# CloudEngineHub/MARL-LLM

Measured on AMD Instinct MI355X. Metric: agent-steps/sec, higher is better.
Workload: dtype f64 (state, every index / flag / reward decision) + f32 (obs, prior, action I/O, pre-filters); 1 GPU; assembly env, 64 agents x 4096 envs per GPU (64 x 4096 total), assembled state, prior-policy actions; agents=64, envs_per_gpu=4096, envs_total=4096, obs_dtype=f32, state_dtype=f64, seed=226, parallelism=env-sharded x1, no collective on the step path

## Files before the change

### marl_llm_amd/csrc/env_api.hip

```cpp

#include <hip/hip_runtime.h>

#include <algorithm>
#include <cmath>
#include <cstddef>
#include <cstdint>
#include <cstring>
#include <new>
#include <string>
#include <utility>
#include <vector>

#include "swarm_env.h"
#include "env_types.h"

using namespace swarm_internal;

namespace {

thread_local std::string g_create_error;

double cut_le(double t) { return cut_lt(std::nextafter(t, INFINITY)); }

int npad_for(int n)
{
    int v = 8;
    while (v < n) v <<= 1;
    return v;
}

int step_launch(swarm_env *h, const Pass &ps)
{
    return h->cfg.large_swarm ? large_launch(h, ps) : env_launch(h, ps);
}

bool detect_lattice(const double *gx, const double *gy, int n, LatEnv &L)
{
    if (n < 2) return false;
    double l2 = INFINITY; int k0 = -1;
    for (int c = 0; c + 1 < n; ++c) {
        const double dx = gx[c + 1] - gx[c], dy = gy[c + 1] - gy[c], d2 = dx * dx + dy * dy;
        if (d2 < l2) { l2 = d2; k0 = c; }
    }
    if (!(l2 > 0) || k0 < 0) return false;
    double cand[4][2]; int ncand = 0;
    for (int c = 0; c + 1 < n && ncand < 4; ++c) {
        const double dx = gx[c + 1] - gx[c], dy = gy[c + 1] - gy[c], d2 = dx * dx + dy * dy;
        if (d2 > l2 * (1.0 + 1e-6)) continue;
        bool seen = false;
        for (int q = 0; q < ncand; ++q)
            if (std::fabs(cand[q][0] - dx) + std::fabs(cand[q][1] - dy) < 1e-6 * std::sqrt(l2)) seen = true;
        if (!seen) { cand[ncand][0] = dx; cand[ncand][1] = dy; ++ncand; }
    }
    std::vector<int> ai((size_t)n), bi((size_t)n);
    double ux = 0, uy = 0, vx = 0, vy = 0;
    bool found = false;
    for (int q = 0; q < ncand && !found; ++q) {
        ux = cand[q][0]; uy = cand[q][1]; vx = -uy; vy = ux;
        for (int pass = 0; pass < 2 && !found; ++pass) {
            bool ok = true;
            for (int c = 0; c < n && ok; ++c) {
                const double rx = gx[c] - gx[0], ry = gy[c] - gy[0];
                const double a = (rx * ux + ry * uy) / l2, b = (rx * vx + ry * vy) / l2;
                const double ar = std::nearbyint(a), br = std::nearbyint(b);
                if (std::fabs(a - ar) > 1e-6 || std::fabs(b - br) > 1e-6 || std::fabs(ar) > 4096 || std::fabs(br) > 4096) ok = false;
                ai[(size_t)c] = (int)ar; bi[(size_t)c] = (int)br;
            }
            if (!ok) break;
            bool order = true, flip = false;
            for (int c = 0; c + 1 < n; ++c) {
                if (bi[(size_t)c + 1] == bi[(size_t)c]) { if (ai[(size_t)c + 1] <= ai[(size_t)c]) order = false; }
                else if (bi[(size_t)c + 1] < bi[(size_t)c]) { flip = true; order = false; }
            }
            if (order) { found = true; break; }
            if (pass == 0 && flip) { vx = -vx; vy = -vy; continue; }
            break;
        }
    }
    if (!found) return false;
    int amin = ai[0], amax = ai[0], bmin = bi[0], bmax = bi[0];
    for (int c = 0; c < n; ++c) {
        amin = std::min(amin, ai[(size_t)c]); amax = std::max(amax, ai[(size_t)c]);
        bmin = std::min(bmin, bi[(size_t)c]); bmax = std::max(bmax, bi[(size_t)c]);
    }
    if (amax - amin + 1 > 64 || bmax - bmin + 1 > 64) return false;
    std::memset(&L, 0, sizeof(L));
    L.ncols = amax - amin + 1; L.nrows = bmax - bmin + 1;
    for (int b = 0; b < 64; ++b) L.rowstart[b] = 0;
    int prev_b = -1;
    for (int c = 0; c < n; ++c) {
        const int a = ai[(size_t)c] - amin, b = bi[(size_t)c] - bmin;
        if (b != prev_b) { if (b < prev_b) return false; L.rowstart[b] = (short)c; prev_b = b; }
        if (L.rowmask[b] & (1ull << a)) return false;
        L.rowmask[b] |= 1ull << a;
    }
    L.ox = gx[0] - (ai[0] - amin) * ux - (bi[0] - bmin) * vx;
    L.oy = gy[0] - (ai[0] - amin) * uy - (bi[0] - bmin) * vy;
    L.uxi = ux / l2; L.uyi = uy / l2; L.vxi = vx / l2; L.vyi = vy / l2;
    const double l = std::sqrt(l2);
    L.R = (float)l;
    return true;
}

int window_rows(float R) { return (int)std::floor(2.0f * (R + 0.01f)) + 1; }

void set_lattice_mode(swarm_env *h, bool any_walk, bool any_scan, float rmax, float cmax, int ncols_max)
{
    KP &k = h->kp;
    if (h->cfg.large_swarm) {
        h->path_mode = PATH_SCAN; h->half = false; k.lattice = 0; k.path_filter = 0;
        return;
    }
    k.lat_n32 = ncols_max <= 32 ? 1 : 0;
    k.lat_rw = (int)std::ceil(rmax + 0.02f);
    k.lat_cw = (int)std::ceil(cmax + 0.02f);
    k.lat_nrs = window_rows(rmax); k.lat_nrc = window_rows(cmax);
    const bool demote = (h->cfg.debug_flags & 8) != 0;
    h->path_mode = (!any_walk || h->lattice_disabled || k.lat_nrs > 15 || (any_scan && demote)) ? PATH_SCAN : any_scan ? PATH_MIXED : PATH_WALK;
    k.lattice = h->path_mode != PATH_SCAN ? 1 : 0;
    k.path_filter = 0;
    {
        const double dx = 1.2e-5, R = std::fmax(1.0, (double)rmax), thr = 0.05 * R / k.d_sen;
        const double dpsi_R = 2.4675 * 2.0 * std::sqrt(2.0) * dx + 1.2e-6 * R;
        k.rew_ga_lat = (float)(1.3 * (dpsi_R + dx + thr * dpsi_R / R));
        k.rew_gb_lat = (float)(4e-6 * R / k.d_sen);
    }
    {
        const int epb_full = env_geometry(h->npad, false).envs;
        const long long grid_full = ((long long)h->cfg.n_env + epb_full - 1) / epb_full;
        h->half = h->path_mode == PATH_WALK && h->npad < 64 && epb_full >= 2 && !(h->cfg.debug_flags & 4) && 2 * grid_full <= (long long)h->n_cu * 6;
    }
    env_layout(k, h->npad, h->half);
}

int export_pass(swarm_env *h, bool lists, bool cap_even)
{
    if (lists && !h->d_exp_occ) {
        const size_t EN = (size_t)h->cfg.n_env * h->cfg.n_agents;
        DevBuf<int> sensed, occ;
        HIP_ALLOC(h, sensed, EN * (size_t)h->kp.g_max);
        HIP_ALLOC(h, occ, EN * (size_t)h->kp.occ_max);
        h->d_exp_sensed = std::move(sensed); h->d_exp_occ = std::move(occ);
    }
    Pass ps;
    ps.export_small = true; ps.export_lists = lists; ps.cap_even = cap_even;
    return step_launch(h, ps);
}

LatInfo classify_cells(const swarm_env *h, const double *gx, const double *gy, int n, LatEnv &L)
{
    std::memset(&L, 0, sizeof(L));
    if (h->lattice_disabled || !detect_lattice(gx, gy, n, L)) {
        std::memset(&L, 0, sizeof(L));
        return LatInfo{false, false, true, 0.0f, 0.0f, 0};
    }
    const double l = L.R;
    L.R = (float)(h->kp.d_sen / l); L.Rc = (float)((h->kp.r_avoid / 2.0) / l);
    const LatInfo info = {true, window_rows(L.R) <= 15, window_rows(L.R) > 15, L.R, L.Rc, L.ncols};
    if (!info.walk) std::memset(&L, 0, sizeof(L));
    return info;
}

LatInfo lattice_summary(const LatInfo *first, const LatInfo *last)
{
    LatInfo m = {true, false, false, 0.0f, 0.0f, 0};
    for (; first != last; ++first) {
        m.ok = m.ok && first->ok; m.scan = m.scan || first->scan;
        if (!first->walk) continue;
        m.walk = true;
        m.R = std::max(m.R, first->R); m.Rc = std::max(m.Rc, first->Rc);
        m.ncols = std::max(m.ncols, first->ncols);
    }
    return m;
}

LatInfo lattice_mode_of(swarm_env *h, const LatInfo *first, const LatInfo *last)
{
    const LatInfo m = lattice_summary(first, last);
    set_lattice_mode(h, m.walk, m.scan, m.R, m.Rc, m.ncols);
    return m;
}

ShapeSet shape_set(const swarm_env *h)
{
    ShapeSet S;
    S.n_shapes = h->n_shapes; S.cells = h->d_shape_cells.get(); S.n_g = h->d_shape_ng.get(); S.l_cell = h->d_shape_l.get();
    S.c_in = h->d_shape_cin.get(); S.lat = h->d_shape_lat.get();
    return S;
}

int interleave(swarm_env *h, int e0, int count)
{
    HIP_LAUNCHED(h, launch_interleave(h->stream, h->d_cells.get(), h->d_cells_xy.get(), h->kp.ng_max, e0, count));
    return SWARM_OK;
}

bool rule_tiled(const swarm_env *h)
{
    return h->cfg.n_agents > 256 || (!h->cfg.large_swarm && (h->cfg.debug_flags & 32) != 0);
}

}

int swarm_internal::fail(swarm_env *h, int code, const std::string &msg)
{
    if (h) h->err = msg; else g_create_error = msg;
    return code;
}

int swarm_internal_env_info(const swarm_env_t *h, swarm_env_info *out)
{
    if (!h || !out) return SWARM_ERR_INVALID;
    out->device = h->device; out->n_env = h->cfg.n_env; out->n_agents = h->cfg.n_agents; out->obs_dim = h->kp.obs_dim;
    out->obs_dtype = h->cfg.obs_dtype; out->with_prior = h->cfg.with_prior != 0; out->observed = h->observed;
    out->g_max = h->kp.g_max; out->llm_action = h->cfg.llm_action != 0; out->n_shapes = h->n_shapes;
    out->large_swarm = h->cfg.large_swarm != 0;
    out->rule_tiled = rule_tiled(h);
    return SWARM_OK;
}

int swarm_internal_metrics_step(swarm_env_t *h, double *out)
{
    if (!h || !out) return SWARM_ERR_INVALID;
    if (!h->have_cells || !h->have_state) return fail(h, SWARM_ERR_STATE, "swarm_rollout_eval: cells / state not set");
    DeviceGuard g(h->device);
    HIP_LAUNCHED(h, launch_metrics_step(h->stream, h->kp, h->n_cu, out));
    return SWARM_OK;
}

int swarm_internal_expert_view(swarm_env_t *h, bool lists, swarm_expert_view *out)
{
    if (!h || !out) return SWARM_ERR_INVALID;
    if (lists) {
        if (!h->d_act64) HIP_ALLOC(h, h->d_act64, (size_t)h->cfg.n_env * h->cfg.n_agents);
        const int rc = export_pass(h, true, true);
        if (rc != SWARM_OK) return rc;
    }
    out->p = h->d_p.get(); out->dp = h->d_dp.get(); out->cells = h->d_cells.get();
    out->near_cell = h->d_near.get(); out->in_flag = h->d_inflag.get(); out->exp_sensed = h->d_exp_sensed.get();
    out->act_next = h->d_act_next.get(); out->act64 = h->d_act64.get();
    out->d_sen = h->kp.d_sen; out->r_avoid = h->kp.r_avoid;
    out->n_env = h->cfg.n_env; out->n_agents = h->cfg.n_agents; out->g_max = h->kp.g_max; out->ng_max = h->kp.ng_max;
    return SWARM_OK;
}

extern "C" {

int swarm_abi_version(void) { return SWARM_ABI_VERSION; }

void swarm_default_config(swarm_config_t *c)
{
    if (!c) return;
    std::memset(c, 0, sizeof(*c));
    c->n_env = 1; c->n_agents = 30; c->n_cells_max = 576;
    c->topo_nei_max = 6; c->num_obs_grid_max = 80; c->num_occupied_grid_max = 200;
    c->is_boundary = 1; c->with_self_state = 1; c->with_prior = 1;
    c->obs_dtype = SWARM_F32; c->device = -1;
    c->d_sen = 0.4; c->r_avoid = 0.15; c->size_a = 0.035;
    c->k_ball = 30; c->k_wall = 100; c->c_wall = 5; c->vel_max = 0.8; c->dt = 0.1;
    c->boundary[0] = -2.4; c->boundary[1] = 2.4; c->boundary[2] = 2.4; c->boundary[3] = -2.4;
    c->prior_gain[0] = 2.0; c->prior_gain[1] = 3.0; c->prior_gain[2] = 2.0;
    c->llm_repulsion = 1.0; c->llm_action = 0;
}

const char *swarm_last_error(const swarm_env_t *h) { return h ? h->err.c_str() : g_create_error.c_str(); }

int swarm_create(const swarm_config_t *cfg, swarm_env_t **out)
{
    if (!cfg || !out) return fail(nullptr, SWARM_ERR_INVALID, "swarm_create: null argument");
    *out = nullptr;
    if (cfg->n_env < 1) return fail(nullptr, SWARM_ERR_INVALID, "n_env must be >= 1");
    if (cfg->large_swarm != 0 && cfg->large_swarm != 1) return fail(nullptr, SWARM_ERR_INVALID, "large_swarm must be 0 or 1");
    if (cfg->large_swarm) {
        if (cfg->n_agents < 1 || cfg->n_agents > 1024) return fail(nullptr, SWARM_ERR_INVALID, "n_agents must be in [1, 1024] (large_swarm)");
    } else if (cfg->n_agents < 1 || cfg->n_agents > 256) return fail(nullptr, SWARM_ERR_INVALID, "n_agents must be in [1, 256]");
    if (cfg->n_cells_max < 1 || cfg->n_cells_max > 32767) return fail(nullptr, SWARM_ERR_INVALID, "n_cells_max must be in [1, 32767]");
    if (cfg->topo_nei_max < 1 || cfg->topo_nei_max > kTopoMax) return fail(nullptr, SWARM_ERR_INVALID, "topo_nei_max must be in [1, 6]");
    if (cfg->num_obs_grid_max < 2 || cfg->num_obs_grid_max > 4096) return fail(nullptr, SWARM_ERR_INVALID, "num_obs_grid_max must be in [2, 4096]");
    if (cfg->num_occupied_grid_max < 2) return fail(nullptr, SWARM_ERR_INVALID, "num_occupied_grid_max must be >= 2");
    if (cfg->obs_dtype != SWARM_F32 && cfg->obs_dtype != SWARM_F64 && cfg->obs_dtype != SWARM_BF16) return fail(nullptr, SWARM_ERR_INVALID, "obs_dtype must be SWARM_F32, SWARM_F64 or SWARM_BF16");
    if (!(cfg->d_sen > 0) || !(cfg->r_avoid > 0) || !(cfg->dt > 0)) return fail(nullptr, SWARM_ERR_INVALID, "d_sen, r_avoid, dt must be positive");

    int ndev = 0;
    hipError_t e = hipGetDeviceCount(&ndev);
    if (e != hipSuccess || ndev < 1)
        return fail(nullptr, SWARM_ERR_HIP, std::string("no HIP device available (") + hipGetErrorString(e) + "); this library has no CPU path");
    int dev = cfg->device;
    if (dev < 0) { if (hipGetDevice(&dev) != hipSuccess) dev = 0; }
    if (dev >= ndev) return fail(nullptr, SWARM_ERR_INVALID, "device ordinal out of range");

    swarm_env *h = new (std::nothrow) swarm_env();
    if (!h) return fail(nullptr, SWARM_ERR_INVALID, "out of host memory");
    h->cfg = *cfg; h->device = dev;
    for (int &a : h->attr_smem) a = -1;
    h->env_lat.assign((size_t)cfg->n_env, LatInfo{false, false, true, 0.0f, 0.0f, 0});
    h->lattice_disabled = (cfg->debug_flags & 2) != 0;
    h->cells_set.assign((size_t)cfg->n_env, 0);
    h->npad = npad_for(cfg->n_agents);

    KP &k = h->kp;
    k.n_env = cfg->n_env; k.n_a = cfg->n_agents; k.ng_max = cfg->n_cells_max;
    k.topo = cfg->topo_nei_max; k.g_max = cfg->num_obs_grid_max; k.occ_max = cfg->num_occupied_grid_max;
    k.with_self = cfg->with_self_state ? 1 : 0;
    k.obs_dim = 2 * 2 * (k.topo + 1 + k.with_self) + 2 * k.g_max;
    k.boundary = cfg->is_boundary ? 1 : 0; k.periodic = cfg->is_boundary ? 0 : 1;
    k.with_prior = cfg->with_prior ? 1 : 0;
    k.pk_att = cfg->prior_gain[0]; k.pk_rep = cfg->prior_gain[1]; k.pk_ali = cfg->prior_gain[2];
    k.pk_llm = cfg->llm_repulsion; k.llm = cfg->llm_action ? 1 : 0;
    k.d_sen = cfg->d_sen; k.r_avoid = cfg->r_avoid; k.size_a = cfg->size_a;
    k.size2 = cfg->size_a + cfg->size_a;
    k.k_ball = cfg->k_ball; k.k_wall = cfg->k_wall; k.c_wall = cfg->c_wall; k.vel_max = cfg->vel_max; k.dt = cfg->dt;
// ... 528 lines not shown
```

### marl_llm_amd/csrc/swarm_env.hip

```cpp

#include <hip/hip_runtime.h>

#include <cmath>
#include <cstdint>
#include <cstring>
#include <string>
#include <type_traits>
#include <utility>

#include "swarm_env.h"
#include "env_types.h"

using namespace swarm_internal;

#if !defined(SWARM_ENV_UNIT)
#define SWARM_UNIT_KERNELS 1
#define SWARM_UNIT_HOST 1
#elif SWARM_ENV_UNIT == 0
#define SWARM_UNIT_KERNELS 0
#define SWARM_UNIT_HOST 1
#else
#define SWARM_UNIT_KERNELS 1
#define SWARM_UNIT_HOST 0
#endif
// ... 187 lines not shown
{
    const bool flip = t > 0.5;
    const double r = flip ? 1.0 - t : t;
    const double x = M_PI * r;
    const double u = x * x;
    double c = -8.8967913924505741e-22;
    c = fma(c, u, 4.1103176233121648e-19);
    c = fma(c, u, -1.5619206968586225e-16);
    c = fma(c, u, 4.7794773323873853e-14);
    c = fma(c, u, -1.1470745597729725e-11);
    c = fma(c, u, 2.0876756987868100e-09);
    c = fma(c, u, -2.7557319223985888e-07);
    c = fma(c, u, 2.4801587301587302e-05);
    c = fma(c, u, -1.3888888888888889e-03);
    c = fma(c, u, 4.1666666666666664e-02);
    c = fma(c, u, -0.5);
    c = fma(c, u, 1.0);
    return flip ? -c : c;
}

__device__ __forceinline__ float psi_u_f32(float u)
{
    float c = 7.969553699e-04f;
    c = fmaf(c, u, -1.267949212e-02f);
    c = fmaf(c, u, 1.175149009e-01f);
    c = fmaf(c, u, -6.675792336e-01f);
    c = fmaf(c, u, 2.029347420e+00f);
    c = fmaf(c, u, -2.467400551e+00f);
    c = fmaf(c, u, 1.0f);
    return c;
}

__device__ __forceinline__ float psi5_u_f32(float u)
{
    float c = -1.028585434e-02f;
    c = fmaf(c, u, 1.148182452e-01f);
    c = fmaf(c, u, -6.661784649e-01f);
    c = fmaf(c, u, 2.029018402e+00f);
    c = fmaf(c, u, -2.467372179e+00f);
    c = fmaf(c, u, 9.999995828e-01f);
    return c;
}

template <bool CAP, int AG>
__device__ __forceinline__ void list_walk_lean(const KP &P, const unsigned *srp, const u64 *rmp, const int aca0, const int k0,
                                               const int k1, const int left, const int nk, float dbf, const float inv_r,
                                               const float apr_s, short *row, float &n0, float &n1, float &dn)
{
    const int G = P.g_max;
    const unsigned nm1 = (unsigned)(nk - 1);
    const unsigned wd0 = *srp;
    u64 rm0 = *rmp;
    srp += AG; ++rmp;
    unsigned nw = *srp;
    u64 nm = *rmp;
    unsigned kept = k0 < k1 ? (wd0 & 0x1FFFFu) : 0u;
    {
        int pb = 0;
#pragma unroll
        for (int sh = 16; sh >= 1; sh >>= 1) {
            const int c = __popc(__builtin_amdgcn_ubfe(kept, 0u, (unsigned)(pb + sh)));
            pb = c <= left ? pb + sh : pb;
        }
        kept = (kept >> pb) << pb;
    }
    int base = (int)(wd0 >> 17);
    unsigned relm = (unsigned)(rm0 >> aca0);
    float db2 = dbf * dbf;
    auto rank_of = [&](int q) -> int {
        if (P.cap_int) {
            const unsigned x = 2u * (unsigned)q * nm1 + (unsigned)(G - 1);
            const unsigned hq_ = __umulhi(x, P.cap_magic);
            return (int)((((x - hq_) >> 1) + hq_) >> P.cap_shift);
        }
        const double v = q * ((double)nm1 / (G - 1));
        return (int)(P.cap_even ? rint(v) : round(v));
    };
    const bool cap = CAP && nk > G;
    int k = k0, slot = k0, nxt = 0;
    if constexpr (CAP) {
        if (cap) {
            if (P.cap_int) slot = k0 > 0 ? (int)((unsigned)((2 * k0 - 1) * (G - 1) + 2 * (int)nm1 - 1) / (2u * nm1)) : 0;
            else {
                slot = 0;
#pragma clang loop vectorize(disable) interleave(disable)
                while (slot < G && rank_of(slot) < k0) ++slot;
            }
            slot = slot < G ? slot : G;
            nxt = slot < G ? rank_of(slot) : 0x7FFFFFFF;
        }
    }
    short *p = row + k0;
    const short *const pend = row + k1;
    typedef float f32x2 __attribute__((ext_vector_type(2)));
    f32x2 n10 = {n1, n0};
    auto more = [&]() -> bool { return CAP ? k < k1 : p < pend; };
    while (__any(more())) {
        if (more()) {
            const int c = __builtin_ctz(kept);
            kept &= kept - 1;
            const int cell = base + __popc(relm & ((1u << c) - 1u));
            const float da = fmaf((float)c, inv_r, -apr_s);
            const float u = fmaf(da, da, db2);
            float psi = psi5_u_f32(u);
            if constexpr (CAP) {
                const bool take = !cap || k == nxt;
                if (take) {
                    row[slot] = (short)cell;
                    ++slot;
                    if (cap) nxt = slot < G ? rank_of(slot) : 0x7FFFFFFF;
                }
                psi = take ? psi : 0.0f;
                ++k;
            } else {
                *p = (short)cell;
                asm volatile("" ::: "memory");
                ++p;
            }
            n10 = __builtin_elementwise_fma(f32x2{psi, psi}, f32x2{dbf, da}, n10); dn += psi;
            asm volatile("" : "+v"(n10), "+v"(dn));
            if (kept == 0) {
                kept = nw & 0x1FFFFu; base = (int)(nw >> 17);
                relm = (unsigned)(nm >> aca0);
                dbf += inv_r;
                if (__builtin_expect(kept == 0, 0)) {
                    while (kept == 0 && more()) {
                        srp += AG; ++rmp;
                        const unsigned wd = *srp;
                        kept = wd & 0x1FFFFu; base = (int)(wd >> 17);
                        relm = (unsigned)(*rmp >> aca0);
                        dbf += inv_r;
                    }
                }
                srp += AG; ++rmp;
                nw = *srp; nm = *rmp;
                db2 = dbf * dbf;
            }
        }
    }
    n1 = n10.x; n0 = n10.y;
}

constexpr float kNoCand = 1e18f;
template <typename MT, int WS>
__device__ __forceinline__ void nearest_rows_lean(const u64 *rm, const short *rs, const int nrows, const int wr, const float apf,
                                                  const float bpf, const int a_r, const MT lowm, const bool act,
                                                  float &best32, float &second32, int &bc)
{
    constexpr int MB = (int)sizeof(MT) * 8;
    auto rowmask = [&](int b) -> MT { return MB == 32 ? (MT)reinterpret_cast<const unsigned *>(rm)[2 * b] : (MT)rm[b]; };
    auto ffbl = [](unsigned v) -> unsigned { unsigned r; asm("v_ffbl_b32 %0, %1" : "=v"(r) : "v"(v)); return r; };
    auto ffbh = [](unsigned v) -> unsigned { unsigned r; asm("v_ffbh_u32 %0, %1" : "=v"(r) : "v"(v)); return r; };
    auto sat = [](unsigned x, unsigned y) -> unsigned { return __builtin_elementwise_add_sat(x, y); };
    int lead = 0, lead_b = 0;
    auto cand_row = [&](int b, MT rowm, auto kc) {
        constexpr int k = decltype(kc)::value;
        const float dy = (float)b - bpf, dy2 = dy * dy;
        const MT up = rowm >> a_r, dn = rowm & lowm;
        unsigned fu, fd;
        if constexpr (MB == 32) { fu = ffbl((unsigned)up); fd = ffbh((unsigned)dn); }
        else {
            fu = min(ffbl((unsigned)up), sat(ffbl((unsigned)((u64)up >> 32)), 32u));
            fd = min(ffbh((unsigned)((u64)dn >> 32)), sat(ffbh((unsigned)dn), 32u));
        }
        const unsigned a_up = sat((unsigned)a_r, fu), a_dn = fd ^ (unsigned)(MB - 1);
        const float dxu = (float)a_up - apf, dxd = (float)a_dn - apf;
        const float d2u = fmaf(dxu, dxu, dy2), d2d = fmaf(dxd, dxd, dy2);
        second32 = __builtin_amdgcn_fmed3f(best32, second32, d2d);
        bool lt = d2d < best32;
        best32 = lt ? d2d : best32; lead = lt ? 2 * k : lead;
        second32 = __builtin_amdgcn_fmed3f(best32, second32, d2u);
        lt = d2u < best32;
        best32 = lt ? d2u : best32; lead = lt ? 2 * k + 1 : lead;
    };
    auto trip = [&](int b, auto tail) {
        constexpr bool TAIL = decltype(tail)::value;
        const MT m0 = rowmask(b), m1 = (!TAIL || b + WS < nrows) ? rowmask(b + WS) : (MT)0;
        const MT m2 = (!TAIL || b + 2 * WS < nrows) ? rowmask(b + 2 * WS) : (MT)0;
        const float best_in = best32;
        cand_row(b, m0, std::integral_constant<int, 0>{}); cand_row(b + WS, m1, std::integral_constant<int, 1>{});
        cand_row(b + 2 * WS, m2, std::integral_constant<int, 2>{});
        if constexpr (!TAIL) cand_row(b + 3 * WS, rowmask(b + 3 * WS), std::integral_constant<int, 3>{});
        lead_b = best32 < best_in ? b : lead_b;
    };
    int b = wr;
    for (; b + 3 * WS < nrows; b += 4 * WS) trip(b, std::false_type{});
    if (b < nrows) trip(b, std::true_type{});
    const bool found = act && best32 < kNoCand;
    const int lrow = found ? lead_b + (lead >> 1) * WS : 0;
    const MT below = rowmask(lrow) & lowm;
    const int lc = rs[lrow] + (MB == 32 ? __popc((unsigned)below) : __popcll((unsigned long long)below)) - 1 + (lead & 1);
    bc = found ? lc : 0;
    if (!act) { best32 = INFINITY; second32 = INFINITY; }
}

template <int NPAD, typename OT, bool DO_STEP, bool LAT, bool HALF = false, bool FILT = false>
__global__ void __launch_bounds__((Geo<NPAD, HALF>::T), (LAT ? Geo<NPAD, HALF>::WPS_LAT : Geo<NPAD, HALF>::WPS_GEN))
k_env(const KP P, const void *__restrict__ action, const int act_mode, OT *__restrict__ obs,
      float *__restrict__ reward, uint8_t *__restrict__ done, OT *__restrict__ a_prior)
{
    typedef Geo<NPAD, HALF> G_;
    constexpr int AG = G_::AG, EPB = G_::EPB, NW = G_::NW, WPE = G_::WPE, T = G_::T;
    constexpr int ACTW = G_::ACTW, LPA = G_::LPA, AGW = G_::AGW;
    static_assert(!HALF || LAT, "the half-occupied geometry exists for the lattice path only");
    static_assert(!HALF || !FILT, "the launches of a mixed batch use the full geometry");
    constexpr bool DIAG = kDiagBuild || !(LAT && NPAD == 64 && !HALF);
    constexpr bool WALK_LEAN = LAT && NPAD == 64 && !HALF;
#ifndef SWARM_WALK_ENV32
#define SWARM_WALK_ENV32 1
#endif
    typedef typename Pair<OT>::type OT2;

    extern __shared__ __align__(16) unsigned char smem[];
    typedef LatMap<NPAD, HALF> LM;
#define LO(r) ((LAT && G_::CT_MAP) ? LM::r : P.off_##r)
    float *cxq = reinterpret_cast<float *>(smem + P.off_cxyf);
    double *sp = reinterpret_cast<double *>(smem + LO(sp));
    u64 *cmask = reinterpret_cast<u64 *>(smem + P.off_cmask);
    float *rsum = reinterpret_cast<float *>(smem + P.off_cmask);
    unsigned *sbits = reinterpret_cast<unsigned *>(smem + P.off_sbits);
    unsigned *obits = reinterpret_cast<unsigned *>(smem + P.off_obits);
    short *sidx = reinterpret_cast<short *>(smem + LO(sidx));
    typedef std::conditional_t<LAT, short, int> pc_t;
    pc_t *part_c = reinterpret_cast<pc_t *>(smem + LO(partc));
    u64 *pm = reinterpret_cast<u64 *>(smem + LO(sidx));
    unsigned *owords = reinterpret_cast<unsigned *>(smem + P.off_cmask);
    short *snei = reinterpret_cast<short *>(smem + LO(snei));
    int *sncf = reinterpret_cast<int *>(smem + LO(sncf));
    u64 *snear = reinterpret_cast<u64 *>(smem + LO(snear));
    u64 *lrm = reinterpret_cast<u64 *>(smem + LO(lat));
    short *lrs = reinterpret_cast<short *>(smem + LO(lat) + (size_t)EPB * 64 * 8);
    int *sflag = reinterpret_cast<int *>(smem + LO(flag));
    unsigned char *pc = smem + P.off_pc;
    constexpr int NRC = LM::NRC;
    float4 *hdr = reinterpret_cast<float4 *>(smem + LO(hdr));
    unsigned *srow = reinterpret_cast<unsigned *>(smem + LO(srow));
    unsigned char *pcr = smem + LO(pcr);
    u64 *covrow = reinterpret_cast<u64 *>(smem + LO(cov));
    unsigned char *perm = smem + LO(perm);
    unsigned *orow = reinterpret_cast<unsigned *>(smem + P.off_orow);

    if constexpr (FILT) {
        bool any_zero = false;
        for (int k = 0; k < EPB; ++k) {
            const int ek = blockIdx.x * EPB + k;
            any_zero = any_zero || P.lat[ek < P.n_env ? ek : P.n_env - 1].nrows == 0;
        }
        if (any_zero == LAT) return;
    }
    const int tid = threadIdx.x, lane = tid & 63;
    STAMP(0);
    const int at = tid % AG;
    const int sx = __builtin_amdgcn_readfirstlane((tid / AG + (int)blockIdx.x) % WPE);
    const int aw = at >> 6;
    auto flag_get = [&]() -> bool { return ((reinterpret_cast<const unsigned *>(sflag)[at >> 2] >> ((at & 3) * 8)) & 1u) != 0; };
    const bool thr_on = NPAD >= 64 || at < ACTW;
    const int el = (NPAD < 64 && thr_on) ? at / NPAD : 0;
    const int i = NPAD < 64 ? at % NPAD : at;
    const int e = blockIdx.x * EPB + el;
    const int n_a = P.n_a;
    const bool act = thr_on && (e < P.n_env) && (i < n_a);
    const int es = e < P.n_env ? e : P.n_env - 1;
    const int ng = P.n_g[es];
    int ngb = ng;
    if (EPB > 1) {
        for (int k = 0; k < EPB; ++k) {
            const int ek = blockIdx.x * EPB + k;
            const int v = P.n_g[ek < P.n_env ? ek : P.n_env - 1];
            ngb = v > ngb ? v : ngb;
        }
    }
    const int W = (ngb + 31) >> 5;
    constexpr int SB = WPE > 1 ? 1 : 0;
    int w0 = W;
    if (WPE > 1) { w0 = (W - 2 * (WPE - 1)) / WPE; w0 = w0 < 0 ? 0 : w0; }
    auto mine = [&](int w) -> bool {
        if (WPE == 1) return true;
        if (w < w0) return sx == SB;
        const int o = (w - w0) % (WPE - 1);
        return sx == (o < SB ? o : o + 1);
    };
    const double2 *gce = P.cells_xy + (size_t)es * P.ng_max;
    auto cell64 = [&](int c) -> double2 { double2 g = gce[c < ng ? c : 0]; if (!(c < ng)) { g.x = kSentinel; g.y = kSentinel; } return g; };
    const float *cq_e = cxq + (size_t)el * P.cxq_stride;

    const size_t sbase = (size_t)es * 2 * n_a;
    double px = __builtin_nan(""), py = __builtin_nan(""), vx = 0.0, vy = 0.0;
    double ax = 0.0, ay = 0.0;
    double sf0x = 0.0, sf0y = 0.0;
    OT2 pri_now; pri_now.x = to_out<OT>(0.0); pri_now.y = to_out<OT>(0.0);
    const bool copy_prior = DO_STEP && P.with_prior && a_prior != nullptr;
    if (sx == 0 && act) {
        if (DO_STEP) { const double2 sfl = P.sf_next[(size_t)e * n_a + i]; sf0x = sfl.x; sf0y = sfl.y; }
        px = P.p[sbase + i]; py = P.p[sbase + n_a + i];
        vx = P.dp[sbase + i]; vy = P.dp[sbase + n_a + i];
        if (DO_STEP) {
            if (act_mode & 2) {
                const size_t a0 = (size_t)e * n_a + i, a1 = a0 + (size_t)P.n_env * n_a;
                if (act_mode & 1) { ax = ((const double *)action)[a0]; ay = ((const double *)action)[a1]; }
                else { ax = (double)((const float *)action)[a0]; ay = (double)((const float *)action)[a1]; }
            }
            else if (act_mode & 1) { const size_t ab = ((size_t)e * n_a + i) * 2; ax = ((const double *)action)[ab]; ay = ((const double *)action)[ab + 1]; }
            else { const float2 af = reinterpret_cast<const float2 *>(action)[(size_t)e * n_a + i]; ax = (double)af.x; ay = (double)af.y; }
            if (copy_prior) pri_now = reinterpret_cast<const OT2 *>(P.prior_next)[(size_t)e * n_a + i];
        }
    }
    if constexpr (!LAT)
    for (int rep = 0, reps = REPS(9); rep < reps; ++rep)
    for (int k = 0; k < EPB; ++k) {
        FENCE();
        const int ek0 = blockIdx.x * EPB + k;
        const int ek = ek0 < P.n_env ? ek0 : P.n_env - 1;
        const int ngk = P.n_g[ek];
        const double *gx = P.cells + (size_t)ek * 2 * P.ng_max;
        const double *gy = gx + P.ng_max;
        for (int c = tid; c < W * 32; c += T) {
            double2 g;
            g.x = c < ngk ? gx[c] : kSentinel;
            g.y = c < ngk ? gy[c] : kSentinel;
            float *q = cxq + (size_t)k * P.cxq_stride + (c >> 1) * 4 + (c & 1);
            q[0] = (float)g.x; q[2] = (float)g.y;
        }
    }
    if (sx == 0) { if constexpr (LAT) { if ((at & 3) == 0) sflag[at >> 2] = 0; } else sflag[at] = 0; }
    if constexpr (LAT) {
        for (int q = tid; q < EPB * 64; q += T) {
            const int ek0 = blockIdx.x * EPB + (q >> 6);
            const LatEnv &Lq = P.lat[ek0 < P.n_env ? ek0 : P.n_env - 1];
            lrm[q] = Lq.rowmask[q & 63]; lrs[q] = Lq.rowstart[q & 63];
            covrow[q] = 0;
        }
        if (sx == WPE - 1) reinterpret_cast<uint4 *>(pcr)[at] = uint4{0u, 0u, 0u, 0u};
    }
    double npx = px, npy = py, nvx = vx, nvy = vy;
    auto forces_integrate = [&]() {
        for (int rep = 0, reps = REPS(1); rep < reps; ++rep) {
            FENCE();
            const double sfx = sf0x, sfy = sf0y;
            STAMP(8);
            double Fx = 1 * ax + sfx, Fy = 1 * ay + sfy;
            if (P.boundary) {
                const double d0 = px - P.size_a - P.bx0;
                const double d1 = P.by1 - (py + P.size_a);
                const double d2 = P.bx2 - (px + P.size_a);
                const double d3 = py - P.size_a - P.by3;
                const double a0 = d0 < 0 ? fabs(d0) : 0.0, a1 = d1 < 0 ? fabs(d1) : 0.0;
// ... 152 lines not shown
#pragma unroll
            for (int w = 0; w < NW; ++w) n1 += __popcll(c1[w]);
            const bool few = n1 >= P.topo;
            if constexpr (NW > 2) {
                u64 c2[NW]; int n2 = 0;
#pragma unroll
                for (int w = 0; w < NW; ++w) c2[w] = cand2N[w];
                if (i < 64 * NW) c2[i >> 6] &= ~(1ull << (i & 63));
#pragma unroll
                for (int w = 0; w < NW; ++w) n2 += __popcll(c2[w]);
                const bool some = n2 >= P.topo;
#pragma unroll
                for (int w = 0; w < NW; ++w) cand[w] = some ? c2[w] : cand[w];
            }
#pragma unroll
            for (int w = 0; w < NW; ++w) cand[w] = few ? c1[w] : cand[w];
        }
        double dmin = INFINITY;
        {
            double nk[kTopoMax + 1];
#pragma unroll
            for (int k = 0; k <= kTopoMax; ++k) nk[k] = INFINITY;
#pragma unroll
            for (int w = 0; w < NW; ++w) {
                u64 h = cand[w];
                while (h) {
                    const int jj = __ffsll((unsigned long long)h) - 1;
                    h &= h - 1;
                    double rx = spx[w * 64 + jj] - px, ry = spy[w * 64 + jj] - py;
                    if (P.periodic) wrap_rel(rx, ry, P.w_half, P.h_half);
                    const double cd = rx * rx + ry * ry;
                    dmin = fmin(dmin, cd);
                    double key = __builtin_bit_cast(double, (__builtin_bit_cast(u64, cd) & ~0xFFull) | (u64)(w * 64 + jj));
#pragma unroll
                    for (int k = 0; k <= kTopoMax; ++k) {
                        const double lo = fmin(nk[k], key);
                        key = fmax(nk[k], key);
                        nk[k] = lo;
                    }
                }
            }
            bool amb = false;
#pragma unroll
            for (int k = 0; k < kTopoMax; ++k) {
                const u64 kb = __builtin_bit_cast(u64, nk[k]), kn = __builtin_bit_cast(u64, nk[k + 1]);
                const bool fin = nk[k] < INFINITY;
                nj[k] = fin ? (int)(kb & 0xFFull) : -1;
                amb = amb || (fin && nk[k + 1] < INFINITY && ((kb ^ kn) >> 8) == 0);
            }
            if (__any(amb)) {
                int xj[kTopoMax];
#pragma unroll
                for (int k = 0; k < kTopoMax; ++k) { nd[k] = INFINITY; xj[k] = -1; }
#pragma unroll
                for (int w = 0; w < NW; ++w) {
                    u64 h = amb ? cand[w] : 0;
                    while (h) {
                        const int jj = __ffsll((unsigned long long)h) - 1;
                        h &= h - 1;
                        double rx = spx[w * 64 + jj] - px, ry = spy[w * 64 + jj] - py;
                        if (P.periodic) wrap_rel(rx, ry, P.w_half, P.h_half);
                        double cd = sqrt(rx * rx + ry * ry); int cj = w * 64 + jj;
                        bool ins = false;
#pragma unroll
                        for (int k = 0; k < kTopoMax; ++k) {
                            const bool sw = ins || cd < nd[k];
                            ins = sw;
                            const double td = nd[k]; const int tjj = xj[k];
                            nd[k] = sw ? cd : td; xj[k] = sw ? cj : tjj;
                            cd = sw ? td : cd;    cj = sw ? tjj : cj;
                        }
                    }
                }
#pragma unroll
                for (int k = 0; k < kTopoMax; ++k) nj[k] = amb ? xj[k] : nj[k];
            }
        }
        STAMP(13);
        if constexpr (NW > 1) {
#pragma unroll
            for (int w = 0; w < NW; ++w) snear[w * AG + at] = nearby[w];
        }
#pragma unroll
        for (int k = 0; k < kTopoMax; ++k) {
            const bool used = k < P.topo && nj[k] >= 0;
            snei[at * kNeiStride + k] = (short)(used ? nj[k] : -1);
            if (P.export_small && act && k < P.topo) P.nei[((size_t)e * n_a + i) * P.topo + k] = used ? nj[k] : -1;
        }
        collision = dmin < P.c_avoid;
        snei[at * kNeiStride + kTopoMax] = (short)(collision ? 1 : 0);
    }
    if (sx == CS) {
        double sfx = 0.0, sfy = 0.0;
        for (int rep = 0, reps = REPS(1); rep < reps; ++rep) {
            FENCE();
            sfx = 0.0; sfy = 0.0;
#pragma unroll
            for (int w = 0; w < NW; ++w) {
                u64 h = hitN[w];
                while (h) {
                    const int kk = __ffsll((unsigned long long)h) - 1;
                    h &= h - 1;
                    const double dx = spx[w * 64 + kk] - px, dy = spy[w * 64 + kk] - py;
                    const double dc = sqrt(dx * dx + dy * dy);
                    const double de = fabs(dc - P.size2);
                    double wx = dx, wy = dy;
                    if (P.periodic) wrap_rel(wx, wy, P.w_half, P.h_half);
                    const double ux = wx / dc, uy = wy / dc;
                    sfx += 1.0 * de * P.k_ball * (-ux);
                    sfy += 1.0 * de * P.k_ball * (-uy);
                }
            }
        }
        if (act) P.sf_next[(size_t)e * n_a + i] = make_double2(sfx, sfy);
        if (NW > 1) __builtin_amdgcn_s_setprio(0);
    }
    STAMP(3);
    EXIT_AT(3);

    const float pxf = (float)px, pyf = (float)py;
    const bool lane_far = act && !(fabs(px) <= (double)P.coord_lim && fabs(py) <= (double)P.coord_lim);
    const bool wave_exact = (P.force_exact != 0) || (__any(lane_far) != 0);
    float best32 = INFINITY, second32 = INFINITY; int bc = 0;
    const f2v pxx = {pxf, pxf}, pyy = {pyf, pyf};
    if constexpr (LAT) {
        if (!(WALK_LEAN && WPE > 1) || sx != SB) {
        const LatEnv &L = P.lat[es];
        const double apd =(px - L.ox) * L.uxi + (py - L.oy) * L.uyi;
        const double bpd = (px - L.ox) * L.vxi + (py - L.oy) * L.vyi;
        const float apf = (float)apd, bpf = (float)bpd;
        const int nrows = L.nrows, ncols = L.ncols;
        const float lat_m = fmaxf(1e-4f, 8e-7f * fmaxf(fabsf(apf), fabsf(bpf)));
        const int b0s = (int)ceilf(bpf - (L.R + 2.0f * lat_m));
        int ca0 = (int)ceilf(apf - (L.R + 2.0f * lat_m));
        ca0 = ca0 < 0 ? 0 : (ca0 > 63 ? 63 : ca0);
        if (sx == 0) {
            float4 hq;
            hq.x = (float)(apd - (double)ca0); hq.y = (float)(bpd - (double)b0s);
            hq.z = __int_as_float(b0s); hq.w = __int_as_float(ca0);
            hdr[at] = hq;
        }
        const u64 *rm = lrm + el * 64;
        const short *rs = lrs + el * 64;
        constexpr int WS = WPE > 1 ? WPE - 1 : 1;
        const int wr = WPE > 1 ? (sx < SB ? sx : sx - 1) : 0;
        auto walk = [&](auto tag) {
        typedef decltype(tag) MT;
        constexpr int MB = (int)sizeof(MT) * 8;
        auto rowmask = [&](int b) -> MT { return MB == 32 ? (MT)reinterpret_cast<const unsigned *>(rm)[2 * b] : (MT)rm[b]; };
        auto popc = [](MT v) -> int { return MB == 32 ? __popc((unsigned)v) : __popcll((unsigned long long)v); };
        auto ffs0 = [](MT v) -> int { return (MB == 32 ? __ffs((unsigned)v) : __ffsll((unsigned long long)v)) - 1; };
        auto range = [](int lo, int hi) -> MT { return hi >= lo ? (MT)((~(MT)0 >> (MB - 1 - hi)) & (~(MT)0 << lo)) : (MT)0; };
        auto row_sel = [&](int b, float rho, double cut) -> MT {
            constexpr bool LEAN = WALK_LEAN;
            const bool rowok = LEAN ? act && (unsigned)b < (unsigned)nrows : act && b >= 0 && b < nrows;
            const float dy = (float)b - bpf, dy2 = dy * dy;
            const float ro = rho + lat_m, ri = rho - lat_m, ri2 = ri > 0.0f ? ri * ri : 0.0f;
            const float ho2 = ro * ro - dy2;
            const bool any_o = rowok && ho2 > 0.0f;
            const float ho = __builtin_amdgcn_sqrtf(LEAN ? __builtin_amdgcn_fmed3f(ho2, 0.0f, INFINITY) : fmaxf(ho2, 0.0f));
            int ao0 = (int)ceilf(apf - ho), ao1 = (int)floorf(apf + ho);
            ao0 = ao0 < 0 ? 0 : ao0; ao1 = ao1 > ncols - 1 ? ncols - 1 : ao1;
            const int bq = b < 0 ? 0 : (b > 63 ? 63 : b);
            const MT rowm = any_o ? rowmask(bq) : (MT)0;
            const int rst = rs[bq];
            const float e0 = (float)ao0 - apf, e1 = (float)ao1 - apf;
            const bool c0 = fmaf(e0, e0, dy2) < ri2, c1 = fmaf(e1, e1, dy2) < ri2;
            MT acc = range(ao0, ao1);
            MT bnd = (MT)((c0 ? (MT)0 : (MT)1 << (ao0 & (MB - 1))) | (c1 ? (MT)0 : (MT)1 << (ao1 & (MB - 1)))) & acc & rowm;
            acc &= ~bnd;
            while (__any(bnd != 0)) {
                if (bnd != 0) {
                    const int a = ffs0(bnd);
                    bnd &= bnd - 1;
                    const int c = rst + popc(rowm & (MT)(((MT)1 << a) - 1));
                    const double2 g = cell64(c);
                    const double ex = g.x - px, ey = g.y - py;
                    if (ex * ex + ey * ey < cut) acc |= (MT)1 << a;
                }
            }
            return rowm & acc;
        };
        for (int rep = 0, reps = REPS(3); rep < reps; ++rep) {
            FENCE();
            for (int t = wr; t < P.lat_nrs; t += WS)
                srow[t * AG + at] = (unsigned)(row_sel(b0s + t, L.R, P.c_sen) >> ca0);
            const int b0c = (int)ceilf(bpf - (L.Rc + 2.0f * lat_m));
            for (int t = wr; t < P.lat_nrc; t += WS) {
                const MT selc = row_sel(b0c + t, L.Rc, P.c_occ);
                const int bq = b0c + t < 0 ? 0 : (b0c + t > 63 ? 63 : b0c + t);
                if (selc != 0) {
                    if constexpr (MB == 32) atomicOr(reinterpret_cast<unsigned *>(&covrow[el * 64 + bq]), (unsigned)selc);
                    else atomicOr(reinterpret_cast<unsigned long long *>(&covrow[el * 64 + bq]), (unsigned long long)selc);
                }
            }
            best32 = INFINITY; second32 = INFINITY; bc = 0;
            const int ar0 = (int)floorf(apf) + 1;
            const int a_r = ar0 < 0 ? 0 : (ar0 > MB - 1 ? MB - 1 : ar0);
            const MT lowm = (MT)(((MT)1 << a_r) - 1);
            const int nr_hi = EPB == 1 ? nrows : 64;
            auto row_cands = [&](int b, float &d2d, float &d2u, int &c_dn) {
                const MT rowm = (EPB == 1 || b < nrows) ? rowmask(b) : (MT)0;
                const float dy = (float)b - bpf, dy2 = dy * dy;
                const MT up = rowm >> a_r, dn = rowm & lowm;
                const int a_up = a_r + ffs0(up);
                const int a_dn = MB - 1 - (MB == 32 ? __clz((int)dn) : __clzll((long long)dn));
                const float dxu = (float)a_up - apf, dxd = (float)a_dn - apf;
                d2u = (act && up != 0) ? fmaf(dxu, dxu, dy2) : INFINITY;
                d2d = (act && dn != 0) ? fmaf(dxd, dxd, dy2) : INFINITY;
                c_dn = rs[b] + popc(dn) - 1;
            };
            float no_cand = INFINITY;
            if constexpr (WALK_LEAN) no_cand = kNoCand;
            if constexpr (WALK_LEAN) {
                nearest_rows_lean<MT, WS>(rm, rs, nrows, wr, apf, bpf, a_r, lowm, act, best32, second32, bc);
            } else
            for (int b = wr; b < nr_hi; b += WS) {
                float d2d, d2u; int c_dn;
                row_cands(b, d2d, d2u, c_dn);
                second32 = __builtin_amdgcn_fmed3f(best32, second32, d2d);
                bool lt = d2d < best32;
                best32 = lt ? d2d : best32; bc = lt ? c_dn : bc;
                second32 = __builtin_amdgcn_fmed3f(best32, second32, d2u);
                lt = d2u < best32;
                best32 = lt ? d2u : best32; bc = lt ? c_dn + 1 : bc;
            }
            const float lat_dlt = 1.2e-7f * fmaxf(fabsf(apf), fabsf(bpf)) + 2e-6f;
            const float tol = 6.0f * sqrtf(second32) * lat_dlt + 1e-9f;
            const bool unc_min = act && (wave_exact || (second32 < no_cand && (second32 - best32) <= tol));
            if (__any(unc_min)) {
                if (unc_min) {
                    const float thr = wave_exact ? INFINITY : best32 + tol;
                    double bestd = INFINITY; int bcd = bc;
                    for (int b = wr; b < nr_hi; b += WS) {
                        float d2d, d2u; int c_dn;
                        row_cands(b, d2d, d2u, c_dn);
                        const bool td = d2d <= thr, tu = d2u <= thr && d2u < INFINITY;
                        if ((td && d2d < INFINITY) || tu) {
                            const double2 g0 = cell64((td && d2d < INFINITY) ? c_dn : 0), g1 = cell64(tu ? c_dn + 1 : 0);
                            const double e0x = g0.x - px, e0y = g0.y - py, e1x = g1.x - px, e1y = g1.y - py;
                            const double q0 = e0x * e0x + e0y * e0y, q1 = e1x * e1x + e1y * e1y;
                            if (td && d2d < INFINITY && q0 < bestd) { bestd = q0; bcd = c_dn; }
                            if (tu && q1 < bestd) { bestd = q1; bcd = c_dn + 1; }
                        }
                    }
                    bc = bcd;
                }
            }
        }
        };
        if (sx != SB || WPE == 1) { if (P.lat_n32 || (WALK_LEAN && SWARM_WALK_ENV32 && ncols <= 32)) walk(0u); else walk((u64)0); }
        }
    } else {
    for (int rep = 0, reps = REPS(3); rep < reps; ++rep) {
    FENCE();
    best32 = INFINITY; second32 = INFINITY; bc = 0;
    for (int w = 0; w < W; ++w) {
        if (!mine(w)) continue;
        unsigned word = 0, rword = 0;
        int mlo = 0, mhi = 0;
        int bl = 0; const float best_in = best32;
        unsigned orw = 0;
        const unsigned nlo = (unsigned)nearby1, nhi = (unsigned)(nearby1 >> 32);
        u64 unc = 0;
        const float4 *cq = reinterpret_cast<const float4 *>(cq_e + w * 64);
        static_for<16>([&](auto prc) {
            constexpr int pr = decltype(prc)::value;
            const float4 q = cq[pr];
            const f2v gx = {q.x, q.y}, gy = {q.z, q.w};
            const f2v rx = gx - pxx, ry = gy - pyy;
            const f2v d2v = __builtin_elementwise_fma(rx, rx, ry * ry);
            static_for<2>([&](auto hc) {
                constexpr int hh = decltype(hc)::value;
                constexpr int b = 2 * pr + hh;
                const float d2 = hh ? d2v.y : d2v.x;
                second32 = __builtin_amdgcn_fmed3f(best32, second32, d2);
                const bool lt = d2 < best32;
                best32 = lt ? d2 : best32;
                bl = lt ? b : bl;
                const u64 m_slo = __ballot(d2 < P.csen_lo), m_shi = __ballot(d2 < P.csen_hi);
                const u64 m_olo = __ballot(d2 < P.cocc_lo), m_ohi = __ballot(d2 < P.cocc_hi);
                rword = shl1_or_mask(rword, m_slo);
                if constexpr (NW == 1) {
                    const unsigned t = ((unsigned)m_olo & nlo) | ((unsigned)(m_olo >> 32) & nhi);
                    orw = shl1_or_mask(orw, __ballot(t != 0));
                } else {
                    mlo = writelane_c<b>((int)(unsigned)m_olo, mlo);
                    mhi = writelane_c<b>((int)(unsigned)(m_olo >> 32), mhi);
                }
                unc |= (m_slo ^ m_shi) | (m_olo ^ m_ohi);
            });
        });
        word = __brev(rword);
        unsigned oword = __brev(orw);
        if (best32 < best_in) bc = w * 32 + bl;
        u64 mym = ((u64)(unsigned)mhi << 32) | (unsigned)mlo;
        if (unc != 0 || wave_exact) {
            word = 0; oword = 0;
#pragma unroll 4
            for (int b = 0; b < 32; ++b) {
                const double2 g = cell64(w * 32 + b);
                const double rx = g.x - px, ry = g.y - py;
                const double d2 = rx * rx + ry * ry;
                if (d2 < P.c_sen) word |= 1u << b;
                const u64 m = __ballot(d2 < P.c_occ);
                if (lane == b) mym = m;
                if (NW == 1 && ((((unsigned)m & nlo) | ((unsigned)(m >> 32) & nhi)) != 0)) oword |= 1u << b;
            }
        }
        sbits[w * AG + at] = word;
        if constexpr (NW == 1) owords[w * AG + at] = oword;
        else if (lane < 32) cmask[(size_t)(w * 32 + lane) * NW + aw] = mym;
    }
    }
    {
        const float tol = P.min_tol_a * sqrtf(second32) + P.min_tol_b * second32 + 1e-9f;
        const bool unc_min = act && (wave_exact || (second32 < INFINITY && (second32 - best32) <= tol));
        if (__any(unc_min)) {
            const float thr = unc_min ? (wave_exact ? INFINITY : best32 + tol) : -1.0f;
            double bestd = INFINITY; int bcd = bc;
            for (int w = 0; w < W; ++w) {
                if (!mine(w)) continue;
                for (int b = 0; b < 32; ++b) {
                    const int cc = w * 32 + b;
                    const float rx = cq_e[(cc >> 1) * 4 + (cc & 1)] - pxf, ry = cq_e[(cc >> 1) * 4 + 2 + (cc & 1)] - pyf;
                    if (fmaf(rx, rx, ry * ry) <= thr || (wave_exact && unc_min)) {
                        const double2 g = cell64(w * 32 + b);
                        const double ex = g.x - px, ey = g.y - py;
                        const double d2 = ex * ex + ey * ey;
                        if (d2 < bestd) { bestd = d2; bcd = w * 32 + b; }
                    }
                }
            }
            if (unc_min) bc = bcd;
        }
    }
    }
    part_c[sx * AG + at] = (pc_t)bc;
    double *part_d = reinterpret_cast<double *>(smem + LO(partd));
    constexpr bool TGT_LDS = LAT && NPAD == 64 && !HALF;
    double2 *tgt = reinterpret_cast<double2 *>(smem + LM::tgt);
    double cand_x = 0.0, cand_y = 0.0;
    int win = 0;
    if constexpr (LAT) {
        if (sx != SB || WPE == 1) {
            const double2 g = cell64(bc);
            const double ex = g.x - px, ey = g.y - py;
            part_d[(WPE > 1 && sx > SB ? sx - 1 : sx) * AG + at] = ex * ex + ey * ey;
            if constexpr (TGT_LDS) { cand_x = ex; cand_y = ey; }
        }
    }
    STAMP(16);
    EXIT_AT(4);
    __syncthreads();
    STAMP(17);
    double best = INFINITY; bc = 0;
    for (int rep = 0, reps = REPS(12); rep < reps; ++rep) {
    FENCE();
    best = INFINITY; bc = 0;
#pragma unroll
    for (int s = 0; s < WPE; ++s) {
        if (LAT && WPE > 1 && s == SB) continue;
        const int c = part_c[s * AG + at];
        double d;
        if constexpr (LAT) d = part_d[(WPE > 1 && s > SB ? s - 1 : s) * AG + at];
        else { const double2 g = cell64(c); const double ex = g.x - px, ey = g.y - py; d = ex * ex + ey * ey; }
        if (d < best || (d == best && c < bc)) { best = d; bc = c; if constexpr (TGT_LDS) win = s; }
    }
    }
    const bool in_shape = act && best < P.c_in[es];
    const bool tgt_mine = TGT_LDS && win == sx;
    if (sx == 0) {
        sncf[at] = bc | (in_shape ? (1 << 30) : 0);
        if (P.export_small && act) {
            P.near_cell[(size_t)e * n_a + i] = bc;
            P.in_flag[(size_t)e * n_a + i] = in_shape ? 1 : 0;
        }
    }
    STAMP(4);
    EXIT_AT(5);

// ... 1158 lines not shown
```

Measured before the change: 3.663 billion agent-steps/s.

## Pack candidate index into float key bits and add lean 32-bit row selection

The nearest-cell search now packs the candidate slot into the low 3 bits of the squared-distance float bits. It then tracks best and second with integer med3/min instead of float med3 plus separate index selects. The tie tolerance is widened to cover the lost mantissa bits. A new lean row-selection routine for the 64-padded lattice walk builds the sensing and coverage row masks relative to the window origin using 32-bit masks, and resolves only the boundary cells exactly in f64. The host also routes configurations with wide coverage windows away from the walk path so the 32-bit masks stay valid. This trims ALU work in the hot walk loop, at the cost of more near-tie fallbacks and some added divergence in the boundary resolution.

```diff
diff --git a/marl_llm_amd/csrc/env_api.hip b/marl_llm_amd/csrc/env_api.hip
--- a/marl_llm_amd/csrc/env_api.hip
+++ b/marl_llm_amd/csrc/env_api.hip
@@ -156,7 +156,8 @@
     }
     const double l = L.R;
     L.R = (float)(h->kp.d_sen / l); L.Rc = (float)((h->kp.r_avoid / 2.0) / l);
-    const LatInfo info = {true, window_rows(L.R) <= 15, window_rows(L.R) > 15, L.R, L.Rc, L.ncols};
+    const bool walks = window_rows(L.R) <= 15 && !(h->npad == 64 && window_rows(L.Rc) > 29);
+    const LatInfo info = {true, walks, !walks, L.R, L.Rc, L.ncols};
     if (!info.walk) std::memset(&L, 0, sizeof(L));
     return info;
 }
diff --git a/marl_llm_amd/csrc/swarm_env.hip b/marl_llm_amd/csrc/swarm_env.hip
--- a/marl_llm_amd/csrc/swarm_env.hip
+++ b/marl_llm_amd/csrc/swarm_env.hip
@@ -363,7 +363,9 @@
     auto ffbl = [](unsigned v) -> unsigned { unsigned r; asm("v_ffbl_b32 %0, %1" : "=v"(r) : "v"(v)); return r; };
     auto ffbh = [](unsigned v) -> unsigned { unsigned r; asm("v_ffbh_u32 %0, %1" : "=v"(r) : "v"(v)); return r; };
     auto sat = [](unsigned x, unsigned y) -> unsigned { return __builtin_elementwise_add_sat(x, y); };
-    int lead = 0, lead_b = 0;
+    auto umed3 = [](unsigned x, unsigned y, unsigned z) -> unsigned { unsigned r; asm("v_med3_u32 %0, %1, %2, %3" : "=v"(r) : "v"(x), "v"(y), "v"(z)); return r; };
+    int lead_b = 0;
+    unsigned kb = __float_as_uint(best32), ks = __float_as_uint(second32);
     auto cand_row = [&](int b, MT rowm, auto kc) {
         constexpr int k = decltype(kc)::value;
         const float dy = (float)b - bpf, dy2 = dy * dy;
@@ -377,32 +379,57 @@
         const unsigned a_up = sat((unsigned)a_r, fu), a_dn = fd ^ (unsigned)(MB - 1);
         const float dxu = (float)a_up - apf, dxd = (float)a_dn - apf;
         const float d2u = fmaf(dxu, dxu, dy2), d2d = fmaf(dxd, dxd, dy2);
-        second32 = __builtin_amdgcn_fmed3f(best32, second32, d2d);
-        bool lt = d2d < best32;
-        best32 = lt ? d2d : best32; lead = lt ? 2 * k : lead;
-        second32 = __builtin_amdgcn_fmed3f(best32, second32, d2u);
-        lt = d2u < best32;
-        best32 = lt ? d2u : best32; lead = lt ? 2 * k + 1 : lead;
+        const unsigned kd = (__float_as_uint(d2d) & ~7u) | (unsigned)(2 * k), ku = (__float_as_uint(d2u) & ~7u) | (unsigned)(2 * k + 1);
+        ks = umed3(kb, ks, kd); kb = min(kb, kd);
+        ks = umed3(kb, ks, ku); kb = min(kb, ku);
     };
     auto trip = [&](int b, auto tail) {
         constexpr bool TAIL = decltype(tail)::value;
         const MT m0 = rowmask(b), m1 = (!TAIL || b + WS < nrows) ? rowmask(b + WS) : (MT)0;
         const MT m2 = (!TAIL || b + 2 * WS < nrows) ? rowmask(b + 2 * WS) : (MT)0;
-        const float best_in = best32;
+        const unsigned kb_in = kb;
         cand_row(b, m0, std::integral_constant<int, 0>{}); cand_row(b + WS, m1, std::integral_constant<int, 1>{});
         cand_row(b + 2 * WS, m2, std::integral_constant<int, 2>{});
         if constexpr (!TAIL) cand_row(b + 3 * WS, rowmask(b + 3 * WS), std::integral_constant<int, 3>{});
-        lead_b = best32 < best_in ? b : lead_b;
+        lead_b = kb < kb_in ? b : lead_b;
     };
     int b = wr;
     for (; b + 3 * WS < nrows; b += 4 * WS) trip(b, std::false_type{});
     if (b < nrows) trip(b, std::true_type{});
+    const int lead = (int)(kb & 7u);
+    best32 = __uint_as_float(kb & ~7u); second32 = __uint_as_float(ks & ~7u);
     const bool found = act && best32 < kNoCand;
     const int lrow = found ? lead_b + (lead >> 1) * WS : 0;
     const MT below = rowmask(lrow) & lowm;
     const int lc = rs[lrow] + (MB == 32 ? __popc((unsigned)below) : __popcll((unsigned long long)below)) - 1 + (lead & 1);
     bc = found ? lc : 0;
     if (!act) { best32 = INFINITY; second32 = INFINITY; }
+}
+
+template <typename MT>
+__device__ __forceinline__ unsigned row_sel_lean(const u64 *rm, const int nrows, const bool act, const int b, const float bpf,
+                                                 const float ax, const int c0, const int cmax, const float ro2, const float ri2,
+                                                 unsigned &bnd)
+{
+    constexpr int MB = (int)sizeof(MT) * 8;
+    auto rowmask = [&](int q) -> MT { return MB == 32 ? (MT)reinterpret_cast<const unsigned *>(rm)[2 * q] : (MT)rm[q]; };
+    const bool rowok = act && (unsigned)b < (unsigned)nrows;
+    const int bq = b < 0 ? 0 : (b > 63 ? 63 : b);
+    const MT rowm = rowmask(bq);
+    const float dy = (float)b - bpf, dy2 = dy * dy;
+    const float ho2 = ro2 - dy2;
+    const float ho = __builtin_amdgcn_sqrtf(__builtin_amdgcn_fmed3f(ho2, 0.0f, INFINITY));
+    const float f0 = ceilf(ax - ho), f1 = floorf(ax + ho);
+    const float lof = fmaxf(f0, 0.0f), hif = fminf(f1, (float)cmax);
+    const int lo = (int)lof, hi = (int)hif;
+    const float e0 = lof - ax, e1 = hif - ax;
+    const bool any_o = rowok && ho2 > 0.0f && hi >= lo;
+    const unsigned wrow = any_o ? (unsigned)(rowm >> (c0 & (MB - 1))) : 0u;
+    const bool ok0 = fmaf(e0, e0, dy2) < ri2, ok1 = fmaf(e1, e1, dy2) < ri2;
+    const unsigned bl = 1u << (lo & 31), bh = 1u << (hi & 31);
+    const unsigned m = ((bh - bl) + bh) & wrow;
+    bnd = ((ok0 ? 0u : bl) | (ok1 ? 0u : bh)) & m;
+    return m ^ bnd;
 }
 
 template <int NPAD, typename OT, bool DO_STEP, bool LAT, bool HALF = false, bool FILT = false>
@@ -861,13 +888,12 @@
         auto ffs0 = [](MT v) -> int { return (MB == 32 ? __ffs((unsigned)v) : __ffsll((unsigned long long)v)) - 1; };
         auto range = [](int lo, int hi) -> MT { return hi >= lo ? (MT)((~(MT)0 >> (MB - 1 - hi)) & (~(MT)0 << lo)) : (MT)0; };
         auto row_sel = [&](int b, float rho, double cut) -> MT {
-            constexpr bool LEAN = WALK_LEAN;
-            const bool rowok = LEAN ? act && (unsigned)b < (unsigned)nrows : act && b >= 0 && b < nrows;
+            const bool rowok = act && b >= 0 && b < nrows;
             const float dy = (float)b - bpf, dy2 = dy * dy;
             const float ro = rho + lat_m, ri = rho - lat_m, ri2 = ri > 0.0f ? ri * ri : 0.0f;
             const float ho2 = ro * ro - dy2;
             const bool any_o = rowok && ho2 > 0.0f;
-            const float ho = __builtin_amdgcn_sqrtf(LEAN ? __builtin_amdgcn_fmed3f(ho2, 0.0f, INFINITY) : fmaxf(ho2, 0.0f));
+            const float ho = __builtin_amdgcn_sqrtf(fmaxf(ho2, 0.0f));
             int ao0 = (int)ceilf(apf - ho), ao1 = (int)floorf(apf + ho);
             ao0 = ao0 < 0 ? 0 : ao0; ao1 = ao1 > ncols - 1 ? ncols - 1 : ao1;
             const int bq = b < 0 ? 0 : (b > 63 ? 63 : b);
@@ -892,6 +918,46 @@
         };
         for (int rep = 0, reps = REPS(3); rep < reps; ++rep) {
             FENCE();
+            if constexpr (WALK_LEAN) {
+                auto lean_row = [&](int b, float ax, int c0, int cmax, float ro2, float ri2, double cut) -> unsigned {
+                    unsigned bnd;
+                    unsigned sel = row_sel_lean<MT>(rm, nrows, act, b, bpf, ax, c0, cmax, ro2, ri2, bnd);
+                    while (__any(bnd != 0)) {
+                        if (bnd != 0) {
+                            const int q = __builtin_ctz(bnd);
+                            bnd &= bnd - 1;
+                            int br = b < 0 ? 0 : (b > 63 ? 63 : b);
+                            asm volatile("" : "+v"(br));
+                            const int c = rs[br] + popc(rowmask(br) & (MT)(((MT)1 << (c0 + q)) - 1));
+                            const double2 g = cell64(c);
+                            const double ex = g.x - px, ey = g.y - py;
+                            if (ex * ex + ey * ey < cut) sel |= 1u << q;
+                        }
+                    }
+                    return sel;
+                };
+                {
+                    const float ax = (float)(apd - (double)ca0);
+                    const int cm = ncols - 1 - ca0, cmax = cm > 30 ? 30 : cm;
+                    const float ro = L.R + lat_m, ri = L.R - lat_m, ro2 = ro * ro, ri2 = ri > 0.0f ? ri * ri : 0.0f;
+                    for (int t = wr; t < P.lat_nrs; t += WS)
+                        srow[t * AG + at] = lean_row(b0s + t, ax, ca0, cmax, ro2, ri2, P.c_sen);
+                }
+                const int b0c = (int)ceilf(bpf - (L.Rc + 2.0f * lat_m));
+                int ca0c = (int)ceilf(apf - (L.Rc + 2.0f * lat_m));
+                ca0c = ca0c < 0 ? 0 : (ca0c > 63 ? 63 : ca0c);
+                const float axc = (float)(apd - (double)ca0c);
+                const int cmc = ncols - 1 - ca0c, cmaxc = cmc > 30 ? 30 : cmc;
+                const float roc = L.Rc + lat_m, ric = L.Rc - lat_m, ro2c = roc * roc, ri2c = ric > 0.0f ? ric * ric : 0.0f;
+                for (int t = wr; t < P.lat_nrc; t += WS) {
+                    const unsigned selc = lean_row(b0c + t, axc, ca0c, cmaxc, ro2c, ri2c, P.c_occ);
+                    const int bq = b0c + t < 0 ? 0 : (b0c + t > 63 ? 63 : b0c + t);
+                    if (selc != 0) {
+                        if constexpr (MB == 32) atomicOr(reinterpret_cast<unsigned *>(&covrow[el * 64 + bq]), selc << (ca0c & 31));
+                        else atomicOr(reinterpret_cast<unsigned long long *>(&covrow[el * 64 + bq]), (unsigned long long)selc << ca0c);
+                    }
+                }
+            } else {
             for (int t = wr; t < P.lat_nrs; t += WS)
                 srow[t * AG + at] = (unsigned)(row_sel(b0s + t, L.R, P.c_sen) >> ca0);
             const int b0c = (int)ceilf(bpf - (L.Rc + 2.0f * lat_m));
@@ -902,6 +968,7 @@
                     if constexpr (MB == 32) atomicOr(reinterpret_cast<unsigned *>(&covrow[el * 64 + bq]), (unsigned)selc);
                     else atomicOr(reinterpret_cast<unsigned long long *>(&covrow[el * 64 + bq]), (unsigned long long)selc);
                 }
+            }
             }
             best32 = INFINITY; second32 = INFINITY; bc = 0;
             const int ar0 = (int)floorf(apf) + 1;
@@ -935,7 +1002,9 @@
                 best32 = lt ? d2u : best32; bc = lt ? c_dn + 1 : bc;
             }
             const float lat_dlt = 1.2e-7f * fmaxf(fabsf(apf), fabsf(bpf)) + 2e-6f;
-            const float tol = 6.0f * sqrtf(second32) * lat_dlt + 1e-9f;
+            float tol_keys = 0.0f;
+            if constexpr (WALK_LEAN) tol_keys = 0x1p-19f * second32;
+            const float tol = 6.0f * sqrtf(second32) * lat_dlt + 1e-9f + tol_keys;
             const bool unc_min = act && (wave_exact || (second32 < no_cand && (second32 - best32) <= tol));
             if (__any(unc_min)) {
                 if (unc_min) {
```

Result: faster. 3.753 billion agent-steps/s, median of 6 (+2.4%).
